# stijnherfst/Tyrant

Hardware: AMD Instinct MI355X
Metric: Mrays/s at 1080p 8spp (higher is better)
Workload: dtype f32

## Files before the change

### include/tyr_c.h

```cpp
#ifndef TYR_C_H
#define TYR_C_H

#include <stddef.h>
#include <stdint.h>

#ifdef __cplusplus
extern "C" {
#endif

#define TYR_ABI_VERSION 5


typedef struct tyr_triangle {
	float vert[3];
	float e1[3];
	float e2[3];
	uint8_t materialType;
	uint8_t pad_[3];
} tyr_triangle;

typedef struct tyr_bbox {
	float bounds[2][3];
} tyr_bbox;

// ... 180 lines not shown
	TYR_TUNE_TICKET_CHUNK = 5,
	TYR_TUNE_STATIC_SHARE = 8,
	TYR_TUNE_STAGED_NODES = 9,
	TYR_TUNE_PROFILE_MASK = 11,
	TYR_TUNE_MERGE_TRACE = 12,
	TYR_TUNE_STATIC_INTERLEAVE = 13,
	TYR_TUNE_RUN_AHEAD = 14,
	TYR_TUNE_WIDE_DRAIN = 15,
	TYR_TUNE_RETIRE_SKY = 20,
	TYR_TUNE_RESOLVE_SHADOWS = 21,
	TYR_TUNE_WIDE_BLOCK_MIN_ITEMS = 22,
	TYR_TUNE_FOLD_PROLOGUE = 23,
	TYR_TUNE_LAYOUT_ON_DEVICE = 24,
	TYR_TUNE_SCAN_IN_TRACE = 25,
	TYR_TUNE_KERNEL_SNAPSHOT = 26,
	TYR_TUNE_FOLD_SPHERES = 19
};
int tyr_set_tuning(tyr_ctx* ctx, int key, int value);

#define TYR_DIST_ID_BYTES 128
typedef struct tyr_dist tyr_dist;
enum {
	TYR_DIST_GATHER = 0,
	TYR_DIST_REDUCE = 1
};
int tyr_dist_unique_id(void* id_out128);
int tyr_dist_create(tyr_dist** out, tyr_ctx* ctx, const void* id128, int32_t rank, int32_t nranks);
int tyr_dist_destroy(tyr_dist* d);
int tyr_dist_combine(tyr_dist* d, int32_t mode, int32_t root, void* frame_out_device);
int tyr_dist_wait(tyr_dist* d);
// ... 130 lines not shown
```

### tyrant_amd/binding.py

```python
from __future__ import annotations

import ctypes as C
import os

import numpy as np

from . import scenes

_HERE = os.path.dirname(os.path.abspath(__file__))
LIB_PATH = os.environ.get("TYRANT_HIP_LIBRARY") or os.path.join(_HERE, "lib", "libtyrant_hip.so")

TYR_FLAG_TRIANGLE_MATERIALS = 1
TYR_FLAG_PROFILE = 2
TYR_FLAG_COUNT_VISITS = 4
TYR_FLAG_LIGHT_LIST = 8
TYR_FLAG_TRIANGLE_COLORS = 16
TYR_FLAG_DEBUG_BVH = 32
TYR_FLAG_REFIT = 64
TYR_ERR_INVALID = -1
TYR_ERR_NO_DEVICE = -2
TYR_ERR_NO_SCENE = -3
TYR_ERR_DEVICE = -6
TYR_ERR_UNSUPPORTED = -7
TYR_QUERY_SPHERES = 1
# ... 392 lines not shown
        return it.value

    def stage(self, name):
        _check(getattr(self.L, "tyr_stage_" + name)(self.h), "tyr_stage_" + name)

    def counters(self) -> dict:
        k = Counters()
        _check(self.L.tyr_get_counters(self.h, C.byref(k)), "tyr_get_counters")
        return k.asdict()

    def timings(self, reset=False) -> dict:
        t = Timings()
        _check(self.L.tyr_get_timings(self.h, C.byref(t), int(reset)), "tyr_get_timings")
        return {n: {"ms": t.ms[i], "launches": int(t.launches[i])} for i, n in enumerate(KERNEL_NAMES)}

    TUNING_KEYS = {"refill_min_idle": 1, "waves_per_simd": 2, "min_traversing": 4, "ticket_chunk": 5, "static_share": 8, "staged_nodes": 9, "profile_mask": 11, "merge_trace": 12, "static_interleave": 13, "run_ahead": 14, "wide_drain": 15, "fold_spheres": 19, "retire_sky": 20, "resolve_shadows": 21, "wide_block_min_items": 22, "fold_prologue": 23, "layout_on_device": 24, "scan_in_trace": 25, "kernel_snapshot": 26}

    def set_tuning(self, **knobs):
        for name, v in knobs.items():
            if v is not None:
                _check(self.L.tyr_set_tuning(self.h, self.TUNING_KEYS[name], int(v)), "tyr_set_tuning")

    def reset_accum(self):
        _check(self.L.tyr_reset_accum(self.h), "tyr_reset_accum")

    def blit_buffer(self) -> np.ndarray:
        out = np.zeros((self.H * self.W, 4), dtype=np.float32)
        _check(self.L.tyr_read_accum(self.h, _ptr(out)), "tyr_read_accum")
        return out

    def resolve_into(self, device_ptr):
# ... 412 lines not shown
```

### tyrant_amd/csrc/hip/adaptive.hip

```cpp
#include <algorithm>
#include <cfloat>

#include "adaptive.hpp"
#include "device_common.hpp"
#include "prologue.hpp"

namespace tyr {

__global__ void __launch_bounds__(kBlock) k_primary_mapped(const FrameParams P, const MappedPrimary M) {
	__shared__ uint32_t baseSh[kClasses], cntSh[8], lastSh;
	const uint32_t index = blockIdx.x * kBlock + threadIdx.x;
	const uint32_t cnt = P.k->primary_ray_cnt;
	const unsigned long long room = (unsigned long long)(P.N - cnt);
	const unsigned long long budget = P.k->budget_remaining;
	const uint32_t nNew = (uint32_t)(room < budget ? room : budget);
	const bool mine = index < nNew;
	const uint32_t vslot = index + cnt;
	uint32_t seed = camera_seed(P, index);

	const bool inList = budget <= (unsigned long long)M.total;
	const uint32_t ticket = M.total - (uint32_t)budget + index;
	const uint32_t p = (mine && inList) ? M.list[ticket] : 0u;
	if (mine && !inList && index == 0u)
		atomicOr(&P.k->device_error, kErrTicketRange);
// ... 408 lines not shown
		const unsigned long long Q = prefix_at(A, A.localPixels - 1u);
		const unsigned long long Qp = prefix_at(A, p), Qq = p ? prefix_at(A, p - 1u) : 0ull;
		const unsigned __int128 E = A.extra;
		const unsigned long long hi = (unsigned long long)((E * Qp) / Q), lo = (unsigned long long)((E * Qq) / Q);
		const unsigned long long want = (unsigned long long)A.minSpp + (hi - lo);
		c = (uint32_t)(want < A.maxSpp ? want : A.maxSpp);
		A.mapOut[frame_index(p, A.W, A.rank, A.nranks)] = c;
	}
	const uint32_t sum = wave_sum_u32(c);
	if ((threadIdx.x & 63u) == 0 && sum)
		atomicAdd(A.totalOut, (unsigned long long)sum);
}


void launch_primary_mapped(const FrameParams& P, const MappedPrimary& M, uint32_t maxNew, hipStream_t stream) {
	hipLaunchKernelGGL(k_primary_mapped, dim3(maxNew ? blocks_for(maxNew) : 1u), dim3(kBlock), 0, stream, P, M);
}
void launch_map_hist(const SampleMapArgs& A, uint32_t localPixels, hipStream_t stream) {
	hipLaunchKernelGGL(k_map_hist, dim3(blocks_for(localPixels)), dim3(kBlock), 0, stream, A, localPixels);
}
void launch_pass_compact(const uint32_t* in, uint32_t n, const uint32_t* counts, uint32_t s, uint32_t* out, uint32_t outLimit, uint32_t* blockCnt, hipStream_t stream) {
	if (n == 0)
		return;
	const uint32_t blocks = (n + kCompactTile - 1) / kCompactTile;
	hipLaunchKernelGGL(k_pass_count, dim3(blocks), dim3(kBlock), 0, stream, in, n, counts, s, blockCnt);
	hipLaunchKernelGGL(k_pass_scan_blocks, dim3(1), dim3(kBlock), 0, stream, blockCnt, blocks);
	hipLaunchKernelGGL(k_pass_scatter, dim3(blocks), dim3(kBlock), 0, stream, in, n, counts, s, out, outLimit, blockCnt);
}
void launch_pass_repeat(uint32_t* list, uint32_t src, uint32_t n, uint32_t dst, uint32_t copies, uint32_t total, hipStream_t stream) {
	const uint32_t len = n * copies;
	if (len != 0)
// ... 15 lines not shown
```

### tyrant_amd/csrc/hip/frame.hip

```cpp
#include "device_common.hpp"
#include "prologue.hpp"

namespace tyr {

__global__ void __launch_bounds__(kBlock) k_primary(const FrameParams P) {
	__shared__ uint32_t baseSh[kClasses], cntSh[8], lastSh;
	const uint32_t index = blockIdx.x * kBlock + threadIdx.x;
	const uint32_t cnt = P.k->primary_ray_cnt;
	const unsigned long long room = (unsigned long long)(P.N - cnt);
	const unsigned long long budget = P.k->budget_remaining;
	const uint32_t nNew = (uint32_t)(room < budget ? room : budget);
	const bool mine = index < nNew;
	const uint32_t vslot = index + cnt;
	uint32_t seed = camera_seed(P, index);

	const uint32_t start = P.k->start_position;
	const int x = (int)((start + index) % P.W);
	const int yl = (int)(((start + index) / P.W) % P.localRows);
	const int y = yl * (int)P.nranks + (int)P.rank;

	const CameraRay cr = camera_lens(P, seed, camera_focus(P, seed, x, y), ld3(P.camPos), ld3(P.camRight), ld3(P.camUp));
	const f3 lensPoint = cr.origin, direction = cr.direction;

	const float2 hitRecord = sphere_hit_record(P, lensPoint, direction);
// ... 106 lines not shown

__global__ void __launch_bounds__(kBlock) k_pad_holes(const FrameParams P, uint32_t workQueue, uint32_t shadowQueue, uint32_t resetTickets) {
	const uint32_t w = blockIdx.x & (kSegs - 1u), what = blockIdx.x / kSegs;
	if (resetTickets && blockIdx.x == 0 && threadIdx.x < kTicketWords)
		P.k->extend_chunks[threadIdx.x * 32] = 0;
	if ((what == 0 && !workQueue) || (what == 1 && !shadowQueue))
		return;
	const uint32_t* cnt = what == 0 ? P.segWork : P.kc->seg;
	const uint32_t mine = cnt[w * kSegStride], ext = queue_extent(cnt) / kSegs;
	for (uint32_t j = mine + threadIdx.x; j < ext; j += kBlock) {
		const uint32_t slot = seg_phys(w, j);
		if (what == 0)
			write_dead_ray(P.work, slot);
		else
			reinterpret_cast<float*>(&P.shadow.color[slot])[3] = 1.0f;
	}
}

__global__ void __launch_bounds__(kBlock) k_connect_spheres(const FrameParams P) {
	const uint32_t first = blockIdx.x * kBlock + threadIdx.x, stride = gridDim.x * kBlock;
	if (first < kTicketWords)
		P.k->extend_chunks[first * 32] = 0;
	__shared__ uint32_t cntSh[kSegs];
	if (threadIdx.x < kSegs)
		cntSh[threadIdx.x] = P.kc->seg[threadIdx.x * kSegStride];
	__syncthreads();
	uint32_t m = 0;
#pragma unroll
	for (uint32_t w = 0; w < kSegs; ++w)
		m = cntSh[w] > m ? cntSh[w] : m;
// ... 220 lines not shown
		P.work.hit[slot] = make_float2(dist, 0.0f);
	}
	float* px = reinterpret_cast<float*>(&P.blit[__float_as_int(P.work.direct_ix[slot].w)]);
	int green = (int)((0.0002f * (float)traversals) * 255.99f);
	green = green > 255 ? 255 : green;
	px[1] = (float)green;
	px[3] = 1.0f;
	if (traversals >= 70) {
		px[0] = (float)green;
		px[1] = 0.0f;
	}
}


constexpr uint32_t kPrepassMaxBlocks = 8192;
void launch_pad_holes(const FrameParams& P, bool workQueue, bool shadowQueue, hipStream_t stream, bool resetTickets) {
	hipLaunchKernelGGL(k_pad_holes, dim3(2 * kSegs), dim3(kBlock), 0, stream, P, workQueue ? 1u : 0u, shadowQueue ? 1u : 0u, resetTickets ? 1u : 0u);
}
void launch_primary(const FrameParams& P, uint32_t maxNew, hipStream_t stream) {
	hipLaunchKernelGGL(k_primary, dim3(maxNew ? blocks_for(maxNew) : 1u), dim3(kBlock), 0, stream, P);
}
void launch_scan(const FrameParams& P, uint32_t maxLive, hipStream_t stream) {
	if (maxLive == 0)
		return;
	hipLaunchKernelGGL(k_scan_words, dim3((maxLive + kScanBlockSlots - 1) / kScanBlockSlots), dim3(kBlock), 0, stream, P);
}
void launch_vecmath_probe(int op, const float* a, const float* b, const float* c, uint32_t n, float* out, hipStream_t stream) {
	hipLaunchKernelGGL(k_vecmath_probe, dim3(blocks_for(n ? n : 1)), dim3(kBlock), 0, stream, op, a, b, c, n, out);
}
void launch_sunsky_probe(const SunParams& S, int which, const float* dirs, uint32_t n, float* out, hipStream_t stream) {
	hipLaunchKernelGGL(k_sunsky_probe, dim3(blocks_for(which == 3 ? 1 : n)), dim3(kBlock), 0, stream, S, which, dirs, n, out);
}
void launch_extend_debug(const FrameParams& P, uint32_t maxLive, hipStream_t stream) {
	if (maxLive != 0)
		hipLaunchKernelGGL(k_extend_debug, dim3(blocks_for(maxLive)), dim3(kBlock), 0, stream, P);
}
void launch_extend_spheres(const FrameParams& P, uint32_t nSurvivors, hipStream_t stream, uint32_t maxLive) {
	const uint32_t walk = std::max(nSurvivors, maxLive);
	if (nSurvivors != 0)
		hipLaunchKernelGGL(k_extend_spheres, dim3(std::min(blocks_for(walk), kPrepassMaxBlocks)), dim3(kBlock), 0, stream, P);
}
void launch_connect_spheres(const FrameParams& P, uint32_t maxShadow, hipStream_t stream) {
	hipLaunchKernelGGL(k_connect_spheres, dim3(std::min(blocks_for(maxShadow), kPrepassMaxBlocks)), dim3(kBlock), 0, stream, P);
}
void launch_resolve(const float4* blit, float4* out, uint32_t nPixels, hipStream_t stream) {
	hipLaunchKernelGGL(k_resolve, dim3(blocks_for(nPixels)), dim3(kBlock), 0, stream, blit, out, nPixels);
}

}
```

### tyrant_amd/csrc/hip/kernels.hpp

```cpp
#pragma once

#include <hip/hip_runtime.h>
#include <stdint.h>

#include "../../../include/tyr_c.h"
#include "sunsky.hpp"
#include "traverse.hpp"

namespace tyr {

struct RayQ {
	float4* o_dx;
	float2* dyz;
	float4* direct_ix;
	uint32_t* flags;
	float2* hit;
	uint32_t* key;
};
constexpr uint32_t kHitSphere = 0x80000000u;
constexpr uint32_t kKeyIndirect = 0x80000000u;
constexpr uint32_t kKeyMask = 0x3fffffffu;
constexpr uint32_t kSegs = 8;
constexpr uint32_t kSegStride = 32;
constexpr uint32_t kClasses = 2;
// ... 122 lines not shown
	int staticShare = 12;
	int staticInterleave = 1;
	int wideDrain = 1;
	int stagedNodes = 64;
	int refillMinIdle = 16;
	int wavesPerSimd = 0;
	int runAhead = 2;
	int mergeTrace = 1;
	int profileMask = 31;
	int resolveShadows = 1;
	int retireSky = 1;
	int wideBlockMinItems = 3 << 20;
	int foldPrologue = 1;
	int layoutOnDevice = 1;
	int scanInTrace = 1;
	int kernelSnapshot = 1;
	int foldSpheres = 1;
};
constexpr uint32_t kCountRaysPerBlock = 1024;

constexpr int kBlock = 256;

enum { kLcShade = 0, kLcTrace, kLcQuery, kLcKinds };
struct LaunchCache {
	int perCU[kLcKinds][6] = {};
};

void launch_primary(const FrameParams& P, uint32_t maxNew, hipStream_t stream);
void launch_pad_holes(const FrameParams& P, bool workQueue, bool shadowQueue, hipStream_t stream, bool resetTickets = false);
void launch_scan(const FrameParams& P, uint32_t maxLive, hipStream_t stream);
void launch_extend(const FrameParams& P, uint32_t maxLive, uint32_t nSurvivors, bool countVisits, const Tuning& t, int numCUs, LaunchCache& lc, hipStream_t stream);
void launch_shade(const FrameParams& P, uint32_t maxLive, int numCUs, LaunchCache& lc, hipStream_t stream);
void launch_trace_prepasses(const FrameParams& P, uint32_t nSurvivors, uint32_t maxShadowPrev, hipStream_t stream, uint32_t maxLive = 0);
void launch_trace_kernel(const FrameParams& P, uint32_t items, const Tuning& t, int numCUs, LaunchCache& lc, hipStream_t stream);
void launch_connect(const FrameParams& P, uint32_t maxShadow, bool countVisits, const Tuning& t, int numCUs, LaunchCache& lc, hipStream_t stream);
void launch_trace(const FrameParams& P, uint32_t maxLive, uint32_t nSurvivors, uint32_t maxShadowPrev, const Tuning& t, int numCUs, LaunchCache& lc, hipStream_t stream);
void launch_extend_spheres(const FrameParams& P, uint32_t nSurvivors, hipStream_t stream, uint32_t maxLive = 0);
void launch_connect_spheres(const FrameParams& P, uint32_t maxShadow, hipStream_t stream);
void launch_resolve(const float4* blit, float4* out, uint32_t nPixels, hipStream_t stream);
void launch_extend_debug(const FrameParams& P, uint32_t maxLive, hipStream_t stream);
void launch_vecmath_probe(int op, const float* a, const float* b, const float* c, uint32_t n, float* out, hipStream_t stream);
// ... 4 lines not shown
```

### tyrant_amd/csrc/hip/shade.hip

```cpp
#include "device_common.hpp"
#include "prologue.hpp"

namespace tyr {

struct ShadeOut {
	bool survive, shadow;
	bool tree;
	f3 origin, direction, direct;
	uint32_t flags;
	f3 sOrigin, sDir, sColor;
	float sClosest;
	f3 color;
	int newFrame;
	float2 hitRec;
	float sBlocked;
	bool sResolved, sVisible;
	bool ghost;
};

struct LightSample {
	f3 toLightUnit, toLight;
	float cosAtSurface, cosAtLight;
	bool valid;
};
// ... 629 lines not shown
			for (uint32_t c = 0; c < kClasses; ++c)
				for (uint32_t w = 0; w < kSegs; ++w)
					PE.k->segSurv[c][w] = __hip_atomic_load(&PE.segNext[c * kClassWords + w * kSegStride], __ATOMIC_RELAXED, __HIP_MEMORY_SCOPE_AGENT);
			lastBlock = true;
			survivors = s;
			snapShadows = h;
		}
	}
	if (PE.shadeOpensNext != 0u) {
		__syncthreads();
		if (tid == 0) {
			sh[16] = (lastBlock && PE.k->n_live != 0u) ? 1u : 0u;
			sh[17] = survivors;
		}
		__syncthreads();
		if (sh[16] != 0u) {
			if (tid < kSegs)
				sh[tid] = __hip_atomic_load(&PE.segNext[tid * kSegStride], __ATOMIC_RELAXED, __HIP_MEMORY_SCOPE_AGENT);
			else if (tid < 2u * kSegs)
				sh[tid] = __hip_atomic_load(&PE.kc->seg[(tid - kSegs) * kSegStride], __ATOMIC_RELAXED, __HIP_MEMORY_SCOPE_AGENT);
			if (tid == 0)
				PE.k->scan_live[PE.scanSet & 1u] = PE.k->n_live;
			__syncthreads();
			pad_work_holes_counts(PE.next, sh);
			pad_shadow_holes_counts(PE.shadow, sh + kSegs);
			__syncthreads();
			wavefront_globals_for(PE, PE.segWork, PE.kcPrev, true, sh[17]);
		}
	}
	if (tid == 0 && lastBlock && PE.hostSnap != nullptr) {
		HostSnap* const hs = PE.hostSnap;
// ... 11 lines not shown
	int* perCU = lc.perCU[kLcShade];
	if (perCU[lights] == 0) {
		int q = 0;
		const hipError_t e = lights ? hipOccupancyMaxActiveBlocksPerMultiprocessor(&q, k_shade<true>, kBlock, 0) : hipOccupancyMaxActiveBlocksPerMultiprocessor(&q, k_shade<false>, kBlock, 0);
		if (e != hipSuccess || q < 1)
			q = 2;
		perCU[lights] = q > 6 ? 6 : q;
	}
	const uint32_t resident = (uint32_t)perCU[lights] * (uint32_t)numCUs;
	return nTiles < resident ? (nTiles ? nTiles : 1u) : resident;
}
void launch_shade(const FrameParams& P0, uint32_t maxSlots, int numCUs, LaunchCache& lc, hipStream_t stream) {
	FrameParams P = P0;
	P.shadeBlocks = shade_grid(P, maxSlots, numCUs, lc);
	if (P.flags & TYR_FLAG_LIGHT_LIST)
		hipLaunchKernelGGL((k_shade<true>), dim3(P.shadeBlocks), dim3(kBlock), 0, stream, P);
	else
		hipLaunchKernelGGL((k_shade<false>), dim3(P.shadeBlocks), dim3(kBlock), 0, stream, P);
}

}
```

### tyrant_amd/csrc/hip/traverse_flat.hip

```cpp
#include "device_common.hpp"
#include "scan_wave.hpp"

namespace tyr {

constexpr uint32_t kTraceBlockWide = 768;
#define TYR_FLAT_WAVES_PER_EU (STACK_LDS <= 8 ? 6 : STACK_LDS <= 12 ? 5 : STACK_LDS <= 16 ? 3 : 2)

__device__ __forceinline__ bool ref_is_leaf(uint32_t ref) { return (ref & kRefLeaf) && ref < kRefPop; }
__device__ __forceinline__ bool ref_is_traversing(uint32_t ref) { return ((int)ref >= 0) || ref == kRefPop; }
__device__ __forceinline__ unsigned long long lanes_traversing(uint32_t ref) { return __builtin_amdgcn_ballot_w64((int)ref >= 0) | __builtin_amdgcn_ballot_w64(ref == kRefPop); }
__device__ __forceinline__ unsigned long long lanes_at_leaf(uint32_t ref) { return __builtin_amdgcn_ballot_w64((ref & kRefLeaf) != 0u) & __builtin_amdgcn_ballot_w64(ref < kRefPop); }

#ifdef TYR_QUAD_STATS
constexpr bool kLoopStats = true;
#else
constexpr bool kLoopStats = false;
#endif
#if defined(TYR_QUAD_STATS) || defined(TYR_LAUNCH_ANATOMY)
constexpr bool kAnatomy = true;
#else
constexpr bool kAnatomy = false;
#endif
#define TYR_DBG(i)                                                     \
	if (COUNT || kLoopStats) {                                         \
// ... 903 lines not shown
		}
	}
}

#undef TYR_DBG
#undef TYR_TRACE_VIEW


#define TYR_TRACE_STACK 12
void launch_trace(const FrameParams& P, uint32_t maxLive, uint32_t nSurvivors, uint32_t maxShadowPrev, const Tuning& t, int numCUs, LaunchCache& lc, hipStream_t stream) {
	launch_trace_prepasses(P, nSurvivors, maxShadowPrev, stream, maxLive);
	launch_trace_kernel(P, maxLive + maxShadowPrev, t, numCUs, lc, stream);
}
void launch_trace_kernel(const FrameParams& P, uint32_t items, const Tuning& t, int numCUs, LaunchCache& lc, hipStream_t stream) {
	if (t.wideBlockMinItems >= 0 && items >= (uint32_t)t.wideBlockMinItems)
		hipLaunchKernelGGL((k_trace_flat<TYR_TRACE_STACK, kTraceBlockWide>), dim3(persistent_blocks(k_trace_flat<TYR_TRACE_STACK, kTraceBlockWide>, items, t, numCUs, lc.perCU[kLcTrace][1], kTraceBlockWide)), dim3(kTraceBlockWide), 0, stream, P);
	else
		hipLaunchKernelGGL((k_trace_flat<TYR_TRACE_STACK, (uint32_t)kBlock>), dim3(persistent_blocks(k_trace_flat<TYR_TRACE_STACK, (uint32_t)kBlock>, items, t, numCUs, lc.perCU[kLcTrace][0])), dim3(kBlock), 0, stream, P);
}
void launch_trace_prepasses(const FrameParams& P, uint32_t nSurvivors, uint32_t maxShadowPrev, hipStream_t stream, uint32_t maxLive) {
	FrameParams Pc = P;
	Pc.kc = P.kcPrev;
	Pc.shadow = P.shadowPrev;
	if (P.prevFolded) {
		if (!P.prologueDone)
			launch_pad_holes(Pc, P.traceShadow != 2u, maxShadowPrev != 0, stream, P.traceShadow == 2u);
		return;
	}
	if (P.traceShadow != 2u)
		launch_extend_spheres(P, nSurvivors, stream, maxLive);
	if (maxShadowPrev != 0)
		launch_connect_spheres(Pc, maxShadowPrev, stream);
	if (P.traceShadow != 2u && nSurvivors == 0)
		launch_pad_holes(Pc, true, false, stream);
}

void launch_extend(const FrameParams& P0, uint32_t maxLive, uint32_t nSurvivors, bool countVisits, const Tuning& t, int numCUs, LaunchCache& lc, hipStream_t stream) {
	if (maxLive == 0)
		return;
	FrameParams P = P0;
	if (countVisits) {
		launch_extend_spheres(P, nSurvivors, stream, maxLive);
		P.raysPerBlock = kCountRaysPerBlock;
		const uint32_t blocks = (P.segCap * kSegs + kCountRaysPerBlock - 1) / kCountRaysPerBlock;
		hipLaunchKernelGGL((k_extend_count<12>), dim3(blocks), dim3(kBlock), 0, stream, P);
		return;
	}
	P.traceShadow = 0u;
	launch_trace(P, maxLive, nSurvivors, 0u, t, numCUs, lc, stream);
}
void launch_connect(const FrameParams& P0, uint32_t maxShadow, bool countVisits, const Tuning& t, int numCUs, LaunchCache& lc, hipStream_t stream) {
	if (maxShadow == 0)
		return;
	FrameParams P = P0;
	if (countVisits) {
		launch_connect_spheres(P, maxShadow, stream);
		P.raysPerBlock = kCountRaysPerBlock;
		const uint32_t blocks = (P.segCap * kSegs + kCountRaysPerBlock - 1) / kCountRaysPerBlock;
		hipLaunchKernelGGL((k_connect_count<12>), dim3(blocks), dim3(kBlock), 0, stream, P);
		return;
	}
	P.kcPrev = P.kc;
	P.shadowPrev = P.shadow;
	P.traceShadow = 2u;
	launch_trace(P, 0u, 0u, maxShadow, t, numCUs, lc, stream);
}

}
```

### tyrant_amd/csrc/host/ctx.hpp

```cpp
#pragma once

#include <vector>

#include <hip/hip_runtime.h>

#include "../hip/refit.hpp"
#include "host.hpp"

using tyr::ConnectCounters;
using tyr::DevCounters;
using tyr::DevScene;
using tyr::LaunchCache;
using tyr::RayQ;
using tyr::ShadowQ;
using tyr::SunParams;
using tyr::Tuning;

struct tyr_ctx {
	tyr_config cfg{};
	hipStream_t stream = nullptr;
	bool ownStream = false;
	uint32_t localRows = 0, localPixels = 0;

	RayQ q[2]{};
// ... 81 lines not shown
	uint32_t svgfCur = 0;
	bool svgfHave = false;

	uint32_t* dTickets = nullptr;
	uint64_t ticketCap = 0;
	uint32_t ticketTotal = 0;
	bool mapped = false;
	uint32_t* dMapScratch = nullptr;
	unsigned long long* dAllocScratch = nullptr;
	hipEvent_t allocDone = nullptr;

	tyr::RefitPlan refit{};

	hipEvent_t ev[2][2 * TYR_K_COUNT]{};
	bool evUsed[2][TYR_K_COUNT]{};
	tyr_timings timings{};
};
```

### tyrant_amd/csrc/host/driver.cpp

```cpp
#include <algorithm>
#include <chrono>
#include <cmath>
#include <cstdio>
#include <cstdlib>
#include <cstring>
#include <new>
#include <thread>
#include <vector>

#include <hip/hip_runtime.h>

#include "../hip/adaptive.hpp"
#include "driver_internal.hpp"

using namespace tyr;
using namespace tyr::drv;

namespace tyr {
namespace drv {

int alloc_rayq(RayQ& q, size_t n) {
	int rc;
	if ((rc = dev_alloc(q.o_dx, n)))
		return rc;
// ... 104 lines not shown
	P.ticketChunk = static_cast<uint32_t>(std::min(std::max(c->tuning.ticketChunk, 64), 65536));
	P.raysPerBlock = tyr::kCountRaysPerBlock;
	P.staticShare = static_cast<uint32_t>(std::min(std::max(c->tuning.staticShare, 0), 15));
	P.staticInterleave = c->tuning.staticInterleave ? 1u : 0u;
	P.wideDrain = c->tuning.wideDrain ? 1u : 0u;
	P.lights = c->dLights;
	P.nLights = c->nLights;
	std::memcpy(P.triEmission, c->triEmission, 12);
	P.palette = c->dPalette;
	return P;
}

struct KernelTimer {
	tyr_ctx* c;
	int k;
	bool on;
	KernelTimer(tyr_ctx* c_, int k_) : c(c_), k(k_), on((c_->cfg.flags & TYR_FLAG_PROFILE) != 0 && ((c_->tuning.profileMask >> k_) & 1) != 0) {
		if (on)
			(void)hipEventRecord(c->ev[c->iter & 1u][2 * k], c->stream);
	}
	~KernelTimer() {
		if (on) {
			(void)hipEventRecord(c->ev[c->iter & 1u][2 * k + 1], c->stream);
			c->evUsed[c->iter & 1u][k] = true;
		}
	}
};
void collect_timings_of(tyr_ctx* c, int set) {
	if (!(c->cfg.flags & TYR_FLAG_PROFILE))
		return;
	for (int k = 0; k < TYR_K_COUNT; ++k) {
		if (!c->evUsed[set][k])
			continue;
		float ms = 0.0f;
		hipError_t e = hipEventElapsedTime(&ms, c->ev[set][2 * k], c->ev[set][2 * k + 1]);
		if (e == hipErrorNotReady) {
			(void)hipGetLastError();
			if (hipEventSynchronize(c->ev[set][2 * k + 1]) == hipSuccess)
				e = hipEventElapsedTime(&ms, c->ev[set][2 * k], c->ev[set][2 * k + 1]);
		}
		if (e == hipSuccess) {
			c->timings.ms[k] += ms;
			c->timings.launches[k] += 1;
		}
		c->evUsed[set][k] = false;
	}
}
void collect_timings(tyr_ctx* c) {
	collect_timings_of(c, 0);
	collect_timings_of(c, 1);
// ... 24 lines not shown
		return TYR_ERR_NO_BUFFER;
	c->firstTime = false;
	camera_basis(c, c->camRight, c->camUp);
	bool reset = false;
	for (int k = 0; k < 3; ++k)
		reset = reset || c->lastPos[k] != c->cam.position[k] || c->lastDir[k] != c->cam.direction[k];
	reset = reset || c->lastFocal != c->cam.focalDistance || c->cam.lensRadius != c->lastLens;
	if (c->sunChanged) {
		c->sunChanged = false;
		reset = true;
		sun_setup(c->sunPos[0], c->sunPos[1], c->sun);
	}
	if (reset) {
		HIPCHK(hipMemsetAsync(c->blit, 0, sizeof(float4) * static_cast<size_t>(c->cfg.width) * c->cfg.height, c->stream));
		c->hK->primary_ray_cnt = 0;
		HIPCHK(hipMemcpyAsync(&c->dK->primary_ray_cnt, &c->hK->primary_ray_cnt, sizeof(uint32_t), hipMemcpyHostToDevice, c->stream));
		std::memset(&c->hK->seg[c->cur][0][0], 0, sizeof c->hK->seg[0]);
		std::memset(c->hK->segSurv, 0, sizeof c->hK->segSurv);
		HIPCHK(hipMemsetAsync(&c->dK->seg[c->cur][0][0], 0, sizeof c->dK->seg[0], c->stream));
		HIPCHK(hipMemsetAsync(c->dK->segSurv, 0, sizeof c->dK->segSurv, c->stream));
	}
	return TYR_OK;
}

void enqueue_primary(tyr_ctx* c, const FrameParams& P, uint32_t nNew) {
	{
		KernelTimer t(c, TYR_K_PRIMARY);
		if (c->mapped)
			launch_primary_mapped(P, MappedPrimary{ c->dTickets, c->ticketTotal }, nNew, c->stream);
		else
			launch_primary(P, nNew, c->stream);
	}
}
void enqueue_extend(tyr_ctx* c, const FrameParams& P0, uint32_t nLive, uint32_t nSurvivors) {
	FrameParams P = P0;
// ... 20 lines not shown
void enqueue_shade(tyr_ctx* c, const FrameParams& P, uint32_t nLive) {
	c->shadowSet = c->iter & 1u;
	c->lastShadeFolded = P.foldSpheres != 0u;
	KernelTimer t(c, TYR_K_SHADE);
	launch_shade(P, nLive, c->numCUs, c->launchCache, c->stream);
	if (P.shadeOpensNext != 0u) {
		c->scanCarried = true;
		c->scanCarriedSet = P.scanSet & 1u;
	} else {
		launch_scan(P, nLive, c->stream);
	}
}
void enqueue_connect(tyr_ctx* c, const FrameParams& P0, uint32_t maxShadow) {
	FrameParams P = P0;
	P.prevFolded = c->lastShadeFolded ? 1u : 0u;
	KernelTimer t(c, TYR_K_CONNECT);
	launch_connect(P, maxShadow, (c->cfg.flags & TYR_FLAG_COUNT_VISITS) != 0, c->tuning, c->numCUs, c->launchCache, c->stream);
}

bool merged_render(const tyr_ctx* c) { return c->tuning.mergeTrace != 0 && !(c->cfg.flags & (TYR_FLAG_COUNT_VISITS | TYR_FLAG_DEBUG_BVH)) && c->scene.rootRef != tyr::kRefDone; }

int flush_pending_shadow(tyr_ctx* c) {
	if (!c->shadowPending)
		return TYR_OK;
	c->shadowPending = false;
	FrameParams P = make_params(c);
	P.kc = P.kcPrev;
	P.shadow = P.shadowPrev;
	enqueue_connect(c, P, c->shadowPendingMax);
	HIPCHK(hipGetLastError());
// ... 546 lines not shown
			return rc;
		c->ownBlit = true;
		HIPCHK(hipMemset(c->blit, 0, n * sizeof(float4)));
	}
	return TYR_OK;
}

void* tyr_get_blit_buffer(tyr_ctx* c) { return c ? c->blit : nullptr; }

int tyr_set_budget(tyr_ctx* c, uint64_t primary_rays) {
	if (!c)
		return TYR_ERR_INVALID;
	int rc = use_device(c);
	if (rc)
		return rc;
	if ((rc = sync_counters(c)))
		return rc;
	c->hK->budget_remaining = primary_rays;
	c->mapped = false;
	return push_counters(c);
}

int tyr_set_frame(tyr_ctx* c, uint32_t frame) {
	if (!c || frame == 0)
		return TYR_ERR_INVALID;
	c->frame = frame;
	return TYR_OK;
}

int tyr_get_counters(tyr_ctx* c, tyr_counters* out) {
	if (!c || !out)
		return TYR_ERR_INVALID;
	int rc = use_device(c);
	if (rc)
		return rc;
// ... 37 lines not shown
	}
	HIPCHK(hipGetLastError());
	HIPCHK(hipStreamSynchronize(c->stream));
	collect_timings(c);
	return TYR_OK;
}

int tyr_reset_accum(tyr_ctx* c) {
	if (!c)
		return TYR_ERR_INVALID;
	if (!c->blit)
		return TYR_ERR_NO_BUFFER;
	int rc = use_device(c);
	if (rc)
		return rc;
	if ((rc = sync_counters(c)))
		return rc;
	HIPCHK(hipMemsetAsync(c->blit, 0, sizeof(float4) * static_cast<size_t>(c->cfg.width) * c->cfg.height, c->stream));
	c->hK->primary_ray_cnt = 0;
	std::memset(&c->hK->seg[c->cur][0][0], 0, sizeof c->hK->seg[0]);
	std::memset(c->hK->segSurv, 0, sizeof c->hK->segSurv);
	return push_counters(c);
}

int tyr_read_accum(tyr_ctx* c, float* host_float4) {
	if (!c || !host_float4)
		return TYR_ERR_INVALID;
	if (!c->blit)
		return TYR_ERR_NO_BUFFER;
	int rc = use_device(c);
	if (rc)
		return rc;
	HIPCHK(hipStreamSynchronize(c->stream));
	HIPCHK(hipMemcpy(host_float4, c->blit, sizeof(float4) * static_cast<size_t>(c->cfg.width) * c->cfg.height, hipMemcpyDeviceToHost));
	return TYR_OK;
}

// ... 83 lines not shown
```

### tyrant_amd/csrc/host/render_loop.cpp

```cpp
#include <algorithm>
#include <chrono>
#include <cmath>
#include <cstdio>
#include <cstdlib>
#include <cstring>
#include <new>
#include <thread>
#include <vector>

#include <hip/hip_runtime.h>

#include "driver_internal.hpp"

using namespace tyr;
using namespace tyr::drv;

extern "C" {

#ifdef TYR_LAUNCH_ANATOMY
static void print_wave_anatomy(const float2* dHit, unsigned long long feedTicks) {
	std::vector<float2> rec(4 * 8192);
	if (hipMemcpy(rec.data(), dHit, rec.size() * sizeof(float2), hipMemcpyDeviceToHost) != hipSuccess)
		return;
	std::vector<float> drain, normal, wide, perTrip, perStep, liveExh, liveWide, trips, steps, passes;
// ... 128 lines not shown

int tyr_launch_kernels(tyr_ctx* c) {
	if (!c)
		return TYR_ERR_INVALID;
	if (!c->haveScene)
		return TYR_ERR_NO_SCENE;
	int rc = use_device(c);
	if (rc)
		return rc;
	return launch_iteration(c, false);
}

struct IterationPlan {
	uint32_t nNew, nLive, nSurvivors, carried;
};
static int enqueue_merged_iteration(tyr_ctx* c, const IterationPlan& p, bool begun, bool foldNext = false, bool prologueDone = false) {
	int rc = begun ? TYR_OK : stage_begin(c);
	if (rc)
		return rc;
	const int set = static_cast<int>(c->iter & 1u);
	FrameParams P = make_params(c);
	if (c->tuning.foldSpheres) {
		P.foldSpheres = 1u;
		P.resolveShadows = c->tuning.resolveShadows ? 1u : 0u;
		P.retireGhosts = (c->tuning.retireSky && c->unboundedRender) ? 1u : 0u;
	}
	if (c->tuning.retireSky)
		P.retireSky = 1u;
	const bool aside = foldNext && c->tuning.scanInTrace != 0;
	P.foldNextPrologue = (foldNext && !aside) ? 1u : 0u;
	P.shadeOpensNext = aside ? 1u : 0u;
	if (aside) {
		P.scanSet = static_cast<uint32_t>(set);
		P.scanLive = &c->dK->scan_live[set];
	}
	P.prologueDone = prologueDone ? 1u : 0u;
	const bool kernelSnap = c->tuning.kernelSnapshot != 0;
	c->snapSeqOf[set] = 0;
	if (kernelSnap) {
		if (++c->snapSeq == 0u)
			++c->snapSeq;
		c->snapSeqOf[set] = c->snapSeq;
		P.hostSnap = c->hostSnapDev[set];
		P.snapSeq = c->snapSeq;
	}
	if (!prologueDone)
		enqueue_primary(c, P, p.nNew);
// ... 38 lines not shown
	uint32_t enq = 1;
	uint32_t lastBirth = 0;
	for (;;) {
		bool ahead = false;
		bool foldedPrev = folded;
		uint32_t frameBefore = c->frame;
		const uint32_t shadowSetBefore = c->shadowSet;
		const bool foldedBefore = c->lastShadeFolded;
		const bool canHaveSurvivors = live != 0 && (budget != 0 || enq - 1 < lastBirth + static_cast<uint32_t>(kMaxBounces));
		if (enq < max_iterations && canHaveSurvivors) {
			const uint32_t liveMax = static_cast<uint32_t>(std::min<uint64_t>(N, static_cast<uint64_t>(live) + budget));
			const uint32_t newMax = static_cast<uint32_t>(std::min<uint64_t>(N, budget));
			const bool opened = folded;
			foldedPrev = folded;
			folded = mayFold && budget == 0 && queued_ahead_behind(enq, 0, lastBirth);
			if ((rc = enqueue_merged_iteration(c, IterationPlan{ newMax, liveMax, live, live }, false, folded, opened))) {
				(void)hipStreamSynchronize(c->stream);
				c->scanCarried = false;
				c->shadowSet = shadowSetBefore;
				c->lastShadeFolded = foldedBefore;
				return rc;
			}
			ahead = true;
		}
		bool flushedEarly = false;
		if (!ahead && mayFold && budget == 0 && !canHaveSurvivors && live != 0) {
			c->shadowPending = true;
			c->shadowPendingMax = live;
			if ((rc = flush_pending_shadow(c)))
				return rc;
			flushedEarly = true;
// ... 93 lines not shown
		if ((rc = use_device(c)))
			return rc;
		rc = render_run_ahead(c, max_iterations, it);
	} else {
		while (it < max_iterations) {
			if ((rc = launch_iteration(c, true)))
				break;
			++it;
			if (c->hK->budget_remaining == 0 && c->hK->primary_ray_cnt == 0)
				break;
		}
	}
	{
		int rcj = rc ? TYR_OK : flush_pending_shadow(c);
		c->shadowPending = false;
		if (!rcj)
			rcj = sync_counters(c);
		if (!rcj)
			collect_timings(c);
		if (c->runAheadUndo) {
			c->runAheadUndo = false;
			if (!rcj) {
				c->hK->n_live = c->undoLive;
				c->hK->shadow_ray_cnt = c->undoShadows;
				rcj = push_counters(c);
			}
		}
		if (!rc)
			rc = rcj ? rcj : check_device_error(c);
	}
	if (iterations_out)
		*iterations_out = it;
	return rc;
}

int tyr_render(tyr_ctx* c, uint32_t spp, uint32_t max_iterations, uint32_t* iterations_out) {
	if (!c)
		return TYR_ERR_INVALID;
	int rc = tyr_set_budget(c, static_cast<uint64_t>(spp) * c->localPixels);
	if (rc)
		return rc;
	if (!c->haveScene)
// ... 17 lines not shown
```

### tyrant_amd/csrc/host/tuning_probes.cpp

```cpp
#include <algorithm>
#include <chrono>
#include <cmath>
#include <cstdio>
#include <cstdlib>
#include <cstring>
#include <new>
#include <thread>
#include <vector>

#include <hip/hip_runtime.h>

#include "driver_internal.hpp"

using namespace tyr;
using namespace tyr::drv;

extern "C" {

int tyr_vecmath_probe(int32_t device, int32_t op, const float* a, const float* b, const float* c, uint32_t n, float* out) {
	if (!a || !b || !c || !out || n == 0 || op < 0 || op > 19)
		return TYR_ERR_INVALID;
	int ndev = 0;
	if (hipGetDeviceCount(&ndev) != hipSuccess || ndev <= 0 || device < 0 || device >= ndev)
		return TYR_ERR_NO_DEVICE;
// ... 173 lines not shown
		{ TYR_TUNE_STATIC_SHARE, 0, 15, &Tuning::staticShare },
		{ TYR_TUNE_STAGED_NODES, 0, static_cast<int>(kStagedNodes), &Tuning::stagedNodes },
		{ TYR_TUNE_PROFILE_MASK, 0, (1 << TYR_K_COUNT) - 1, &Tuning::profileMask },
		{ TYR_TUNE_MERGE_TRACE, 0, 1, &Tuning::mergeTrace },
		{ TYR_TUNE_STATIC_INTERLEAVE, 0, 1, &Tuning::staticInterleave },
		{ TYR_TUNE_RUN_AHEAD, 0, 2, &Tuning::runAhead },
		{ TYR_TUNE_WIDE_DRAIN, 0, 1, &Tuning::wideDrain },
		{ TYR_TUNE_FOLD_SPHERES, 0, 1, &Tuning::foldSpheres },
		{ TYR_TUNE_RETIRE_SKY, 0, 1, &Tuning::retireSky },
		{ TYR_TUNE_RESOLVE_SHADOWS, 0, 1, &Tuning::resolveShadows },
		{ TYR_TUNE_WIDE_BLOCK_MIN_ITEMS, -1, 0x7fffffff, &Tuning::wideBlockMinItems },
		{ TYR_TUNE_FOLD_PROLOGUE, 0, 1, &Tuning::foldPrologue },
		{ TYR_TUNE_LAYOUT_ON_DEVICE, 0, 1, &Tuning::layoutOnDevice },
		{ TYR_TUNE_SCAN_IN_TRACE, 0, 1, &Tuning::scanInTrace },
		{ TYR_TUNE_KERNEL_SNAPSHOT, 0, 1, &Tuning::kernelSnapshot },
	};
	for (const Knob& k : knobs) {
		if (k.key != key)
			continue;
		if (value < k.lo || value > k.hi)
			return TYR_ERR_INVALID;
		c->tuning.*(k.field) = value;
		return TYR_OK;
	}
	return TYR_ERR_INVALID;
}

int tyr_get_timings(tyr_ctx* c, tyr_timings* out, int reset) {
	if (!c || !out)
		return TYR_ERR_INVALID;
// ... 8 lines not shown
```

Before: 8293.

## Replace host counter syncs with device poke kernel and carry final scan into connect

Host-side sync_counters/push_counters round trips and memset/memcpy pairs used to reset queues, set the budget and undo run-ahead are replaced by one tiny device kernel that writes the counters in stream order. The last merged iteration of a render now has shade do the scan-prologue work (shadeOpensNext=2), and connect picks up the carried scan state, removing a separate prologue step. An optional stage-timing mode attaches events to kernel launches through hipExtLaunchKernelGGL, off by default. This removes host stalls and launches, but counter updates now depend on correct device ordering and the end-of-render path becomes more complex.

```diff
diff --git a/include/tyr_c.h b/include/tyr_c.h
--- a/include/tyr_c.h
+++ b/include/tyr_c.h
@@ -218,6 +218,7 @@
 	TYR_TUNE_LAYOUT_ON_DEVICE = 24,
 	TYR_TUNE_SCAN_IN_TRACE = 25,
 	TYR_TUNE_KERNEL_SNAPSHOT = 26,
+	TYR_TUNE_STAGE_TIMING = 27,
 	TYR_TUNE_FOLD_SPHERES = 19
 };
 int tyr_set_tuning(tyr_ctx* ctx, int key, int value);
diff --git a/tyrant_amd/binding.py b/tyrant_amd/binding.py
--- a/tyrant_amd/binding.py
+++ b/tyrant_amd/binding.py
@@ -430,7 +430,7 @@
         _check(self.L.tyr_get_timings(self.h, C.byref(t), int(reset)), "tyr_get_timings")
         return {n: {"ms": t.ms[i], "launches": int(t.launches[i])} for i, n in enumerate(KERNEL_NAMES)}
 
-    TUNING_KEYS = {"refill_min_idle": 1, "waves_per_simd": 2, "min_traversing": 4, "ticket_chunk": 5, "static_share": 8, "staged_nodes": 9, "profile_mask": 11, "merge_trace": 12, "static_interleave": 13, "run_ahead": 14, "wide_drain": 15, "fold_spheres": 19, "retire_sky": 20, "resolve_shadows": 21, "wide_block_min_items": 22, "fold_prologue": 23, "layout_on_device": 24, "scan_in_trace": 25, "kernel_snapshot": 26}
+    TUNING_KEYS = {"refill_min_idle": 1, "waves_per_simd": 2, "min_traversing": 4, "ticket_chunk": 5, "static_share": 8, "staged_nodes": 9, "profile_mask": 11, "merge_trace": 12, "static_interleave": 13, "run_ahead": 14, "wide_drain": 15, "fold_spheres": 19, "retire_sky": 20, "resolve_shadows": 21, "wide_block_min_items": 22, "fold_prologue": 23, "layout_on_device": 24, "scan_in_trace": 25, "kernel_snapshot": 26, "stage_timing": 27}
 
     def set_tuning(self, **knobs):
         for name, v in knobs.items():
diff --git a/tyrant_amd/csrc/hip/adaptive.hip b/tyrant_amd/csrc/hip/adaptive.hip
--- a/tyrant_amd/csrc/hip/adaptive.hip
+++ b/tyrant_amd/csrc/hip/adaptive.hip
@@ -446,7 +446,7 @@
 
 
 void launch_primary_mapped(const FrameParams& P, const MappedPrimary& M, uint32_t maxNew, hipStream_t stream) {
-	hipLaunchKernelGGL(k_primary_mapped, dim3(maxNew ? blocks_for(maxNew) : 1u), dim3(kBlock), 0, stream, P, M);
+	launch_in_stage(k_primary_mapped, dim3(maxNew ? blocks_for(maxNew) : 1u), dim3(kBlock), stream, P, M);
 }
 void launch_map_hist(const SampleMapArgs& A, uint32_t localPixels, hipStream_t stream) {
 	hipLaunchKernelGGL(k_map_hist, dim3(blocks_for(localPixels)), dim3(kBlock), 0, stream, A, localPixels);
diff --git a/tyrant_amd/csrc/hip/frame.hip b/tyrant_amd/csrc/hip/frame.hip
--- a/tyrant_amd/csrc/hip/frame.hip
+++ b/tyrant_amd/csrc/hip/frame.hip
@@ -144,6 +144,26 @@
 			write_dead_ray(P.work, slot);
 		else
 			reinterpret_cast<float*>(&P.shadow.color[slot])[3] = 1.0f;
+	}
+}
+
+__global__ void __launch_bounds__(kBlock) k_poke_counters(DevCounters* __restrict__ k, const CounterPoke p) {
+	if (p.what & kPokeResetQueue) {
+		uint32_t* const seg = &k->seg[p.queue & 1u][0][0];
+		for (uint32_t i = threadIdx.x; i < kClasses * kSegs * kSegStride; i += kBlock)
+			seg[i] = 0u;
+		if (threadIdx.x < kClasses * kSegs)
+			(&k->segSurv[0][0])[threadIdx.x] = 0u;
+		if (threadIdx.x == 0)
+			k->primary_ray_cnt = 0u;
+	}
+	if (threadIdx.x == 0) {
+		if (p.what & kPokeBudget)
+			k->budget_remaining = p.budget;
+		if (p.what & kPokeLiveShadow) {
+			k->n_live = p.nLive;
+			k->shadow_ray_cnt = p.shadows;
+		}
 	}
 }
 
@@ -394,16 +414,23 @@
 
 
 constexpr uint32_t kPrepassMaxBlocks = 8192;
+StageEvents*& open_stage_events() {
+	static thread_local StageEvents* open = nullptr;
+	return open;
+}
+void launch_poke_counters(DevCounters* k, const CounterPoke& p, hipStream_t stream) {
+	hipLaunchKernelGGL(k_poke_counters, dim3(1), dim3(kBlock), 0, stream, k, p);
+}
 void launch_pad_holes(const FrameParams& P, bool workQueue, bool shadowQueue, hipStream_t stream, bool resetTickets) {
-	hipLaunchKernelGGL(k_pad_holes, dim3(2 * kSegs), dim3(kBlock), 0, stream, P, workQueue ? 1u : 0u, shadowQueue ? 1u : 0u, resetTickets ? 1u : 0u);
+	launch_in_stage(k_pad_holes, dim3(2 * kSegs), dim3(kBlock), stream, P, workQueue ? 1u : 0u, shadowQueue ? 1u : 0u, resetTickets ? 1u : 0u);
 }
 void launch_primary(const FrameParams& P, uint32_t maxNew, hipStream_t stream) {
-	hipLaunchKernelGGL(k_primary, dim3(maxNew ? blocks_for(maxNew) : 1u), dim3(kBlock), 0, stream, P);
+	launch_in_stage(k_primary, dim3(maxNew ? blocks_for(maxNew) : 1u), dim3(kBlock), stream, P);
 }
 void launch_scan(const FrameParams& P, uint32_t maxLive, hipStream_t stream) {
 	if (maxLive == 0)
 		return;
-	hipLaunchKernelGGL(k_scan_words, dim3((maxLive + kScanBlockSlots - 1) / kScanBlockSlots), dim3(kBlock), 0, stream, P);
+	launch_in_stage(k_scan_words, dim3((maxLive + kScanBlockSlots - 1) / kScanBlockSlots), dim3(kBlock), stream, P);
 }
 void launch_vecmath_probe(int op, const float* a, const float* b, const float* c, uint32_t n, float* out, hipStream_t stream) {
 	hipLaunchKernelGGL(k_vecmath_probe, dim3(blocks_for(n ? n : 1)), dim3(kBlock), 0, stream, op, a, b, c, n, out);
@@ -413,18 +440,18 @@
 }
 void launch_extend_debug(const FrameParams& P, uint32_t maxLive, hipStream_t stream) {
 	if (maxLive != 0)
-		hipLaunchKernelGGL(k_extend_debug, dim3(blocks_for(maxLive)), dim3(kBlock), 0, stream, P);
+		launch_in_stage(k_extend_debug, dim3(blocks_for(maxLive)), dim3(kBlock), stream, P);
 }
 void launch_extend_spheres(const FrameParams& P, uint32_t nSurvivors, hipStream_t stream, uint32_t maxLive) {
 	const uint32_t walk = std::max(nSurvivors, maxLive);
 	if (nSurvivors != 0)
-		hipLaunchKernelGGL(k_extend_spheres, dim3(std::min(blocks_for(walk), kPrepassMaxBlocks)), dim3(kBlock), 0, stream, P);
+		launch_in_stage(k_extend_spheres, dim3(std::min(blocks_for(walk), kPrepassMaxBlocks)), dim3(kBlock), stream, P);
 }
 void launch_connect_spheres(const FrameParams& P, uint32_t maxShadow, hipStream_t stream) {
-	hipLaunchKernelGGL(k_connect_spheres, dim3(std::min(blocks_for(maxShadow), kPrepassMaxBlocks)), dim3(kBlock), 0, stream, P);
+	launch_in_stage(k_connect_spheres, dim3(std::min(blocks_for(maxShadow), kPrepassMaxBlocks)), dim3(kBlock), stream, P);
 }
 void launch_resolve(const float4* blit, float4* out, uint32_t nPixels, hipStream_t stream) {
-	hipLaunchKernelGGL(k_resolve, dim3(blocks_for(nPixels)), dim3(kBlock), 0, stream, blit, out, nPixels);
-}
-
-}
+	launch_in_stage(k_resolve, dim3(blocks_for(nPixels)), dim3(kBlock), stream, blit, out, nPixels);
+}
+
+}
diff --git a/tyrant_amd/csrc/hip/kernels.hpp b/tyrant_amd/csrc/hip/kernels.hpp
--- a/tyrant_amd/csrc/hip/kernels.hpp
+++ b/tyrant_amd/csrc/hip/kernels.hpp
@@ -1,6 +1,7 @@
 #pragma once
 
 #include <hip/hip_runtime.h>
+#include <hip/hip_ext.h>
 #include <stdint.h>
 
 #include "../../../include/tyr_c.h"
@@ -160,6 +161,7 @@
 	int foldPrologue = 1;
 	int layoutOnDevice = 1;
 	int scanInTrace = 1;
+	int stageTiming = 0;
 	int kernelSnapshot = 1;
 	int foldSpheres = 1;
 };
@@ -171,6 +173,37 @@
 struct LaunchCache {
 	int perCU[kLcKinds][6] = {};
 };
+
+enum : uint32_t {
+	kPokeResetQueue = 1u,
+	kPokeBudget = 2u,
+	kPokeLiveShadow = 4u,
+};
+struct CounterPoke {
+	uint32_t what = 0u;
+	uint32_t queue = 0u;
+	uint32_t nLive = 0u, shadows = 0u;
+	unsigned long long budget = 0ull;
+};
+void launch_poke_counters(DevCounters* k, const CounterPoke& p, hipStream_t stream);
+
+struct StageEvents {
+	hipEvent_t start = nullptr, stop = nullptr;
+	uint32_t launches = 0u;
+};
+StageEvents*& open_stage_events();
+#if defined(__HIPCC__)
+template <class... KArgs, class... Args>
+inline void launch_in_stage(void (*kernel)(KArgs...), dim3 grid, dim3 block, hipStream_t stream, Args&&... args) {
+	StageEvents* const se = open_stage_events();
+	if (!se) {
+		hipLaunchKernelGGL(kernel, grid, block, 0, stream, static_cast<Args&&>(args)...);
+		return;
+	}
+	hipExtLaunchKernelGGL(kernel, grid, block, 0, stream, se->launches == 0u ? se->start : nullptr, se->stop, 0, static_cast<Args&&>(args)...);
+	se->launches++;
+}
+#endif
 
 void launch_primary(const FrameParams& P, uint32_t maxNew, hipStream_t stream);
 void launch_pad_holes(const FrameParams& P, bool workQueue, bool shadowQueue, hipStream_t stream, bool resetTickets = false);
diff --git a/tyrant_amd/csrc/hip/shade.hip b/tyrant_amd/csrc/hip/shade.hip
--- a/tyrant_amd/csrc/hip/shade.hip
+++ b/tyrant_amd/csrc/hip/shade.hip
@@ -667,7 +667,16 @@
 			sh[17] = survivors;
 		}
 		__syncthreads();
-		if (sh[16] != 0u) {
+		if (sh[16] != 0u && PE.shadeOpensNext == 2u) {
+			if (tid < kSegs)
+				sh[kSegs + tid] = __hip_atomic_load(&PE.kc->seg[tid * kSegStride], __ATOMIC_RELAXED, __HIP_MEMORY_SCOPE_AGENT);
+			if (tid < kTicketWords)
+				PE.k->extend_chunks[tid * 32] = 0;
+			if (tid == 0)
+				PE.k->scan_live[PE.scanSet & 1u] = PE.k->n_live;
+			__syncthreads();
+			pad_shadow_holes_counts(PE.shadow, sh + kSegs);
+		} else if (sh[16] != 0u) {
 			if (tid < kSegs)
 				sh[tid] = __hip_atomic_load(&PE.segNext[tid * kSegStride], __ATOMIC_RELAXED, __HIP_MEMORY_SCOPE_AGENT);
 			else if (tid < 2u * kSegs)
@@ -709,9 +718,9 @@
 	FrameParams P = P0;
 	P.shadeBlocks = shade_grid(P, maxSlots, numCUs, lc);
 	if (P.flags & TYR_FLAG_LIGHT_LIST)
-		hipLaunchKernelGGL((k_shade<true>), dim3(P.shadeBlocks), dim3(kBlock), 0, stream, P);
+		launch_in_stage((k_shade<true>), dim3(P.shadeBlocks), dim3(kBlock), stream, P);
 	else
-		hipLaunchKernelGGL((k_shade<false>), dim3(P.shadeBlocks), dim3(kBlock), 0, stream, P);
+		launch_in_stage((k_shade<false>), dim3(P.shadeBlocks), dim3(kBlock), stream, P);
 }
 
 }
diff --git a/tyrant_amd/csrc/hip/traverse_flat.hip b/tyrant_amd/csrc/hip/traverse_flat.hip
--- a/tyrant_amd/csrc/hip/traverse_flat.hip
+++ b/tyrant_amd/csrc/hip/traverse_flat.hip
@@ -941,9 +941,9 @@
 }
 void launch_trace_kernel(const FrameParams& P, uint32_t items, const Tuning& t, int numCUs, LaunchCache& lc, hipStream_t stream) {
 	if (t.wideBlockMinItems >= 0 && items >= (uint32_t)t.wideBlockMinItems)
-		hipLaunchKernelGGL((k_trace_flat<TYR_TRACE_STACK, kTraceBlockWide>), dim3(persistent_blocks(k_trace_flat<TYR_TRACE_STACK, kTraceBlockWide>, items, t, numCUs, lc.perCU[kLcTrace][1], kTraceBlockWide)), dim3(kTraceBlockWide), 0, stream, P);
+		launch_in_stage((k_trace_flat<TYR_TRACE_STACK, kTraceBlockWide>), dim3(persistent_blocks(k_trace_flat<TYR_TRACE_STACK, kTraceBlockWide>, items, t, numCUs, lc.perCU[kLcTrace][1], kTraceBlockWide)), dim3(kTraceBlockWide), stream, P);
 	else
-		hipLaunchKernelGGL((k_trace_flat<TYR_TRACE_STACK, (uint32_t)kBlock>), dim3(persistent_blocks(k_trace_flat<TYR_TRACE_STACK, (uint32_t)kBlock>, items, t, numCUs, lc.perCU[kLcTrace][0])), dim3(kBlock), 0, stream, P);
+		launch_in_stage((k_trace_flat<TYR_TRACE_STACK, (uint32_t)kBlock>), dim3(persistent_blocks(k_trace_flat<TYR_TRACE_STACK, (uint32_t)kBlock>, items, t, numCUs, lc.perCU[kLcTrace][0])), dim3(kBlock), stream, P);
 }
 void launch_trace_prepasses(const FrameParams& P, uint32_t nSurvivors, uint32_t maxShadowPrev, hipStream_t stream, uint32_t maxLive) {
 	FrameParams Pc = P;
@@ -970,7 +970,7 @@
 		launch_extend_spheres(P, nSurvivors, stream, maxLive);
 		P.raysPerBlock = kCountRaysPerBlock;
 		const uint32_t blocks = (P.segCap * kSegs + kCountRaysPerBlock - 1) / kCountRaysPerBlock;
-		hipLaunchKernelGGL((k_extend_count<12>), dim3(blocks), dim3(kBlock), 0, stream, P);
+		launch_in_stage((k_extend_count<12>), dim3(blocks), dim3(kBlock), stream, P);
 		return;
 	}
 	P.traceShadow = 0u;
@@ -984,7 +984,7 @@
 		launch_connect_spheres(P, maxShadow, stream);
 		P.raysPerBlock = kCountRaysPerBlock;
 		const uint32_t blocks = (P.segCap * kSegs + kCountRaysPerBlock - 1) / kCountRaysPerBlock;
-		hipLaunchKernelGGL((k_connect_count<12>), dim3(blocks), dim3(kBlock), 0, stream, P);
+		launch_in_stage((k_connect_count<12>), dim3(blocks), dim3(kBlock), stream, P);
 		return;
 	}
 	P.kcPrev = P.kc;
diff --git a/tyrant_amd/csrc/host/ctx.hpp b/tyrant_amd/csrc/host/ctx.hpp
--- a/tyrant_amd/csrc/host/ctx.hpp
+++ b/tyrant_amd/csrc/host/ctx.hpp
@@ -119,5 +119,6 @@
 
 	hipEvent_t ev[2][2 * TYR_K_COUNT]{};
 	bool evUsed[2][TYR_K_COUNT]{};
+	bool evEmpty[2][TYR_K_COUNT]{};
 	tyr_timings timings{};
 };
diff --git a/tyrant_amd/csrc/host/driver.cpp b/tyrant_amd/csrc/host/driver.cpp
--- a/tyrant_amd/csrc/host/driver.cpp
+++ b/tyrant_amd/csrc/host/driver.cpp
@@ -1,4 +1,5 @@
 #include <algorithm>
+#include <cassert>
 #include <chrono>
 #include <cmath>
 #include <cstdio>
@@ -142,15 +143,27 @@
 struct KernelTimer {
 	tyr_ctx* c;
 	int k;
-	bool on;
-	KernelTimer(tyr_ctx* c_, int k_) : c(c_), k(k_), on((c_->cfg.flags & TYR_FLAG_PROFILE) != 0 && ((c_->tuning.profileMask >> k_) & 1) != 0) {
-		if (on)
+	bool on, attached;
+	tyr::StageEvents se;
+	KernelTimer(tyr_ctx* c_, int k_) : c(c_), k(k_), on((c_->cfg.flags & TYR_FLAG_PROFILE) != 0 && ((c_->tuning.profileMask >> k_) & 1) != 0), attached(on && c_->tuning.stageTiming != 0) {
+		if (attached) {
+			assert(tyr::open_stage_events() == nullptr);
+			se.start = c->ev[c->iter & 1u][2 * k];
+			se.stop = c->ev[c->iter & 1u][2 * k + 1];
+			tyr::open_stage_events() = &se;
+		} else if (on) {
 			(void)hipEventRecord(c->ev[c->iter & 1u][2 * k], c->stream);
+		}
 	}
 	~KernelTimer() {
-		if (on) {
+		if (attached) {
+			tyr::open_stage_events() = nullptr;
+			c->evUsed[c->iter & 1u][k] = true;
+			c->evEmpty[c->iter & 1u][k] = se.launches == 0u;
+		} else if (on) {
 			(void)hipEventRecord(c->ev[c->iter & 1u][2 * k + 1], c->stream);
 			c->evUsed[c->iter & 1u][k] = true;
+			c->evEmpty[c->iter & 1u][k] = false;
 		}
 	}
 };
@@ -161,7 +174,7 @@
 		if (!c->evUsed[set][k])
 			continue;
 		float ms = 0.0f;
-		hipError_t e = hipEventElapsedTime(&ms, c->ev[set][2 * k], c->ev[set][2 * k + 1]);
+		hipError_t e = c->evEmpty[set][k] ? hipSuccess : hipEventElapsedTime(&ms, c->ev[set][2 * k], c->ev[set][2 * k + 1]);
 		if (e == hipErrorNotReady) {
 			(void)hipGetLastError();
 			if (hipEventSynchronize(c->ev[set][2 * k + 1]) == hipSuccess)
@@ -216,11 +229,13 @@
 	if (reset) {
 		HIPCHK(hipMemsetAsync(c->blit, 0, sizeof(float4) * static_cast<size_t>(c->cfg.width) * c->cfg.height, c->stream));
 		c->hK->primary_ray_cnt = 0;
-		HIPCHK(hipMemcpyAsync(&c->dK->primary_ray_cnt, &c->hK->primary_ray_cnt, sizeof(uint32_t), hipMemcpyHostToDevice, c->stream));
 		std::memset(&c->hK->seg[c->cur][0][0], 0, sizeof c->hK->seg[0]);
 		std::memset(c->hK->segSurv, 0, sizeof c->hK->segSurv);
-		HIPCHK(hipMemsetAsync(&c->dK->seg[c->cur][0][0], 0, sizeof c->dK->seg[0], c->stream));
-		HIPCHK(hipMemsetAsync(c->dK->segSurv, 0, sizeof c->dK->segSurv, c->stream));
+		tyr::CounterPoke p;
+		p.what = tyr::kPokeResetQueue;
+		p.queue = static_cast<uint32_t>(c->cur);
+		launch_poke_counters(c->dK, p, c->stream);
+		HIPCHK(hipGetLastError());
 	}
 	return TYR_OK;
 }
@@ -271,6 +286,13 @@
 void enqueue_connect(tyr_ctx* c, const FrameParams& P0, uint32_t maxShadow) {
 	FrameParams P = P0;
 	P.prevFolded = c->lastShadeFolded ? 1u : 0u;
+	if (c->scanCarried) {
+		P.prologueDone = 1u;
+		P.scanPrevInTrace = 1u;
+		P.scanLivePrev = &c->dK->scan_live[c->scanCarriedSet];
+		P.retireGhosts = (c->tuning.foldSpheres && c->tuning.retireSky && c->unboundedRender) ? 1u : 0u;
+		c->scanCarried = false;
+	}
 	KernelTimer t(c, TYR_K_CONNECT);
 	launch_connect(P, maxShadow, (c->cfg.flags & TYR_FLAG_COUNT_VISITS) != 0, c->tuning, c->numCUs, c->launchCache, c->stream);
 }
@@ -847,11 +869,14 @@
 	int rc = use_device(c);
 	if (rc)
 		return rc;
-	if ((rc = sync_counters(c)))
-		return rc;
 	c->hK->budget_remaining = primary_rays;
 	c->mapped = false;
-	return push_counters(c);
+	tyr::CounterPoke p;
+	p.what = tyr::kPokeBudget;
+	p.budget = primary_rays;
+	launch_poke_counters(c->dK, p, c->stream);
+	HIPCHK(hipGetLastError());
+	return TYR_OK;
 }
 
 int tyr_set_frame(tyr_ctx* c, uint32_t frame) {
@@ -919,13 +944,16 @@
 	int rc = use_device(c);
 	if (rc)
 		return rc;
-	if ((rc = sync_counters(c)))
-		return rc;
 	HIPCHK(hipMemsetAsync(c->blit, 0, sizeof(float4) * static_cast<size_t>(c->cfg.width) * c->cfg.height, c->stream));
 	c->hK->primary_ray_cnt = 0;
 	std::memset(&c->hK->seg[c->cur][0][0], 0, sizeof c->hK->seg[0]);
 	std::memset(c->hK->segSurv, 0, sizeof c->hK->segSurv);
-	return push_counters(c);
+	tyr::CounterPoke p;
+	p.what = tyr::kPokeResetQueue;
+	p.queue = static_cast<uint32_t>(c->cur);
+	launch_poke_counters(c->dK, p, c->stream);
+	HIPCHK(hipGetLastError());
+	return TYR_OK;
 }
 
 int tyr_read_accum(tyr_ctx* c, float* host_float4) {
diff --git a/tyrant_amd/csrc/host/render_loop.cpp b/tyrant_amd/csrc/host/render_loop.cpp
--- a/tyrant_amd/csrc/host/render_loop.cpp
+++ b/tyrant_amd/csrc/host/render_loop.cpp
@@ -166,7 +166,7 @@
 struct IterationPlan {
 	uint32_t nNew, nLive, nSurvivors, carried;
 };
-static int enqueue_merged_iteration(tyr_ctx* c, const IterationPlan& p, bool begun, bool foldNext = false, bool prologueDone = false) {
+static int enqueue_merged_iteration(tyr_ctx* c, const IterationPlan& p, bool begun, bool foldNext = false, bool prologueDone = false, bool endsRender = false) {
 	int rc = begun ? TYR_OK : stage_begin(c);
 	if (rc)
 		return rc;
@@ -182,7 +182,10 @@
 	const bool aside = foldNext && c->tuning.scanInTrace != 0;
 	P.foldNextPrologue = (foldNext && !aside) ? 1u : 0u;
 	P.shadeOpensNext = aside ? 1u : 0u;
-	if (aside) {
+	const bool closes = endsRender && !foldNext && c->tuning.scanInTrace != 0;
+	if (closes)
+		P.shadeOpensNext = 2u;
+	if (aside || closes) {
 		P.scanSet = static_cast<uint32_t>(set);
 		P.scanLive = &c->dK->scan_live[set];
 	}
@@ -251,7 +254,8 @@
 			const bool opened = folded;
 			foldedPrev = folded;
 			folded = mayFold && budget == 0 && queued_ahead_behind(enq, 0, lastBirth);
-			if ((rc = enqueue_merged_iteration(c, IterationPlan{ newMax, liveMax, live, live }, false, folded, opened))) {
+			const bool endsRender = mayFold && budget == 0 && !(enq < lastBirth + static_cast<uint32_t>(kMaxBounces));
+			if ((rc = enqueue_merged_iteration(c, IterationPlan{ newMax, liveMax, live, live }, false, folded, opened, endsRender))) {
 				(void)hipStreamSynchronize(c->stream);
 				c->scanCarried = false;
 				c->shadowSet = shadowSetBefore;
@@ -375,18 +379,21 @@
 	{
 		int rcj = rc ? TYR_OK : flush_pending_shadow(c);
 		c->shadowPending = false;
+		if (c->runAheadUndo) {
+			c->runAheadUndo = false;
+			if (!rcj) {
+				tyr::CounterPoke p;
+				p.what = tyr::kPokeLiveShadow;
+				p.nLive = c->undoLive;
+				p.shadows = c->undoShadows;
+				launch_poke_counters(c->dK, p, c->stream);
+				rcj = static_cast<int>(hipGetLastError());
+			}
+		}
 		if (!rcj)
 			rcj = sync_counters(c);
 		if (!rcj)
 			collect_timings(c);
-		if (c->runAheadUndo) {
-			c->runAheadUndo = false;
-			if (!rcj) {
-				c->hK->n_live = c->undoLive;
-				c->hK->shadow_ray_cnt = c->undoShadows;
-				rcj = push_counters(c);
-			}
-		}
 		if (!rc)
 			rc = rcj ? rcj : check_device_error(c);
 	}
diff --git a/tyrant_amd/csrc/host/tuning_probes.cpp b/tyrant_amd/csrc/host/tuning_probes.cpp
--- a/tyrant_amd/csrc/host/tuning_probes.cpp
+++ b/tyrant_amd/csrc/host/tuning_probes.cpp
@@ -211,6 +211,7 @@
 		{ TYR_TUNE_LAYOUT_ON_DEVICE, 0, 1, &Tuning::layoutOnDevice },
 		{ TYR_TUNE_SCAN_IN_TRACE, 0, 1, &Tuning::scanInTrace },
 		{ TYR_TUNE_KERNEL_SNAPSHOT, 0, 1, &Tuning::kernelSnapshot },
+		{ TYR_TUNE_STAGE_TIMING, 0, 1, &Tuning::stageTiming },
 	};
 	for (const Knob& k : knobs) {
 		if (k.key != key)
```

Result: faster. 8403 (median of 6 runs) (+1.3%).
